# AhmedSalih3d/SPHExample

Hardware: AMD Instinct MI355X
Metric: particle-updates/sec (3D dam-break) (higher is better)
Workload: dtype f32

## Files before the change

sphexample_amd/csrc/sphmi_engine.hip:

```cpp
#include <hip/hip_runtime.h>

#include <algorithm>
#include <cmath>
#include <cstdio>
#include <cstring>
#include <limits>
#include <stdexcept>
#include <string>
#include <vector>

#include "../../include/sphmi.h"
#include "../../include/sphmi_internal.h"
#include "sphmi_kernels.h"
#include "sphmi_rebuild.h"

namespace sphmi {

struct EngineError : std::runtime_error {
    int status;
    EngineError(int s, const std::string& m) : std::runtime_error(m), status(s) {}
};

#define HC(expr)                                                                                   \
    do {                                                                                           \
// ... 220 lines not shown
        xcd_trace = getenv("SPHMI_XCD_TRACE") != nullptr;
        if (const char* w = getenv("SPHMI_TPB")) { const int v = atoi(w); if (v == 1 || v == 2 || v == 4) tpb = v; }
        if (const char* w = getenv("SPHMI_RESCHED")) resched = atoi(w);
        if (const char* w = getenv("SPHMI_TPB2")) tpb2 = atoi(w);
        if (const char* w = getenv("SPHMI_WPT2_BELOW")) kWptMedium = atoi(w);
        if (const char* w = getenv("SPHMI_CLASSES_FINE_BELOW")) classes_fine_below = atoi(w);
        HC(hipMalloc(&xcd_clock_d, 16 * 8)); HC(hipHostMalloc(&xcd_clock_h, 32 * 8));
        if (const char* w = getenv("SPHMI_XCD_SEGS")) { const int v = atoi(w); if (v >= 1 && v <= 4096) xcd_segs = v; }
        const size_t n = (size_t)N;
        for (int k = 0; k < 3; ++k) { HC(hipMalloc(&rec[k], 2 * n * sizeof(V4))); pk0[k] = Half<V4>(rec[k]); pk1[k] = Half<V4>(rec[k] + 1); }
        for (int k = 0; k < 2; ++k) {
            HC(hipMalloc(&acc[k], n * sizeof(V4)));
            HC(hipMalloc(&ghost[k], n * sizeof(V4))); HC(hipMemset(ghost[k], 0, n * sizeof(V4)));
            HC(hipMalloc(&type[k], n));
            HC(hipMalloc(&id[k], n * 8));
            HC(hipMalloc(&grp[k], n * 8));
            HC(hipMalloc(&key[k], n * 4));
            HC(hipMalloc(&prow[k], n * 4));
        }
        {
            const char* w = getenv("SPHMI_COMPENSATE");
            if (sizeof(T) == 4 && !(w && atoi(w) == 0))
                for (int k = 0; k < 2; ++k) { HC(hipMalloc(&comp[k], n * sizeof(V4))); HC(hipMemset(comp[k], 0, n * sizeof(V4))); }
        }
        HC(hipMalloc(&slot, n * 4)); HC(hipMalloc(&tmp_idx, n * 4)); HC(hipMalloc(&perm, n * 4));
        if (const char* w = getenv("SPHMI_POISON")) {
            const int b = atoi(w) & 255;
            for (int k = 0; k < 3; ++k) HC(hipMemset(rec[k], b, 2 * n * sizeof(V4)));
            for (int k = 0; k < 2; ++k) HC(hipMemset(acc[k], b, n * sizeof(V4)));
        }
        const size_t nt = n / kWave + 2;
        for (int k = 0; k < 2; ++k) { HC(hipMalloc(&tile_cost[k], nt * 4)); HC(hipMalloc(&tile_order[k], 8 * nt * 4)); }
        HC(hipMalloc(&tile_scan, nt * 4)); HC(hipMalloc(&tile_cls, nt)); HC(hipMalloc(&tile_work_d, nt * 4)); HC(hipMalloc(&tile_work1_d, nt * 4));
        if (cfg.kernel_output == SPHMI_KOUT_STORE) { HC(hipMalloc(&kout_d, n * sizeof(V4))); HC(hipMemset(kout_d, 0, n * sizeof(V4))); }
#if defined(SPHMI_STATS) || defined(SPHMI_TRACE)
        HC(hipMalloc(&trace_d, nt * 32 * 9)); HC(hipMemset(trace_d, 0, nt * 32 * 9));
#endif
        HC(hipMalloc(&tile_tsum, (nt / kScanTile + 2) * 4));
        static_assert(2 * sizeof(StepCtrl) <= kCtlRed, "control block layout");
        HC(hipMalloc(&ctl_d, kCtlBytes)); HC(hipMemset(ctl_d, 0, kCtlBytes)); HC(hipHostMalloc(&ctl_m, kCtlBytes)); memset(ctl_m, 0, kCtlBytes);
        ctrl_d = (StepCtrl*)ctl_d; red_d = (unsigned long long*)(ctl_d + kCtlRed); misc_d = (int*)(ctl_d + kCtlMisc); part_d = (int*)(ctl_d + kCtlPart);
        red_h = (unsigned long long*)(ctl_m + kCtlRed); misc_h = (int*)(ctl_m + kCtlMisc); part_h = (int*)(ctl_m + kCtlPart);
        HC(hipHostMalloc(&ctrl_h, sizeof(StepCtrl)));
        if (const char* w = getenv("SPHMI_FUSE_CTRL")) fuse_ctrl = atoi(w);
        if (const char* w = getenv("SPHMI_FUSE_MDBC")) fuse_mdbc = atoi(w);
        if (const char* w = getenv("SPHMI_SAME_CELLS")) same_cells = atoi(w);
        if (const char* w = getenv("SPHMI_DEVICE_REBUILD")) dev_rebuild = atoi(w);
        HC(hipMalloc(&bbox_d, 8 * 4));
        HC(hipHostMalloc(&bbox_h, 8 * 4));
    }
    ~Engine() override {
        (void)hipSetDevice(cfg.device);
        if (stream) (void)hipStreamSynchronize(stream);
        for (auto& e : ev_pool) { (void)hipEventDestroy(e.a); (void)hipEventDestroy(e.b); }
        for (auto& e : ev_pending) { (void)hipEventDestroy(e.a); (void)hipEventDestroy(e.b); }
        for (int k = 0; k < 3; ++k) (void)hipFree(rec[k]);
        for (int k = 0; k < 2; ++k) {
            (void)hipFree(acc[k]); (void)hipFree(ghost[k]); (void)hipFree(type[k]); (void)hipFree(id[k]); (void)hipFree(otag[k]);
            (void)hipFree(grp[k]); (void)hipFree(key[k]); (void)hipFree(prow[k]); (void)hipFree(comp[k]);
        }
        if (copy_stream) { (void)hipStreamSynchronize(copy_stream); (void)hipStreamDestroy(copy_stream); (void)hipEventDestroy(ev_packed); }
        for (auto& e : host_pinned) (void)hipHostUnregister(e.first);
        (void)hipFree(out_arena);
        (void)hipFree(slot); (void)hipFree(tmp_idx); (void)hipFree(perm);
        for (int k = 0; k < 2; ++k) { (void)hipFree(tile_cost[k]); (void)hipFree(tile_order[k]); }
        (void)hipFree(kout_d); (void)hipFree(tile_work_d); (void)hipFree(tile_work1_d); (void)hipFree(xcd_clock_d); (void)hipHostFree(xcd_clock_h);
        (void)hipFree(tile_scan); (void)hipFree(tile_cls); (void)hipFree(tile_tsum);
        (void)hipFree(count); (void)hipFree(cstart); (void)hipFree(tsum);
#if defined(SPHMI_STATS) || defined(SPHMI_TRACE)
        if (trace_d) {
            const char* fn = getenv("SPHMI_TRACE_FILE");
            std::vector<unsigned long long> tr((size_t)(cap / kWave + 2) * 4 * 9);
            if (fn && hipMemcpy(tr.data(), trace_d, tr.size() * 8, hipMemcpyDeviceToHost) == hipSuccess) {
                FILE* f = fopen(fn, "wb");
                if (f) { fwrite(tr.data(), 8, tr.size(), f); fclose(f); }
            }
            (void)hipFree(trace_d);
        }
#endif
#ifdef SPHMI_STATS
        {
            unsigned long long st[16];
            if (hipMemcpy(st, red_d, sizeof st, hipMemcpyDeviceToHost) == hipSuccess)
                fprintf(stderr, "[sphmi stats] wave-iterations %llu  lane-iterations %llu  refills %llu  empty refills %llu  chunks %llu  waves %llu\n",
                        st[8], st[9], st[10], st[11], st[12], st[13]);
        }
#endif
        (void)hipFree(ctl_d); (void)hipHostFree(ctl_m); (void)hipHostFree(ctrl_h); (void)hipFree(mdbc_list_d);
        (void)hipFree(bbox_d);
        (void)hipHostFree(bbox_h);
        (void)hipFree(cellx_d); (void)hipFree(uc_tsum);
        if (stream && own_stream) (void)hipStreamDestroy(stream);
    }

    static constexpr int kEvSample = 8;
    int ev_period = kEvSample;
    Ev begin_phase(int phase) {
        Ev e{};
        e.phase = phase; e.bstep = batch_step;
        e.weight = (phase == PH_REBUILD || phase == PH_REBUILD_DEVICE || iteration < ev_always_until) ? 1 : ((iteration % ev_period) == 0 ? ev_period : 0);
        if (e.weight == 0) return e;
        if (!ev_pool.empty()) { const int w = e.weight; e = ev_pool.back(); ev_pool.pop_back(); e.phase = phase; e.weight = w; e.bstep = batch_step; }
        else {
            HC(hipEventCreateWithFlags(&e.a, hipEventDisableSystemFence)); HC(hipEventCreateWithFlags(&e.b, hipEventDisableSystemFence));
        }
        HC(hipEventRecord(e.a, stream));
        return e;
    }
    void end_phase(Ev e) { if (e.weight == 0) return; HC(hipEventRecord(e.b, stream)); ev_pending.push_back(e); }
    void collect_events(int64_t executed = INT64_MAX) {
        for (auto& e : ev_pending) {
            float ms = 0;
            if (e.bstep >= 0 && e.bstep >= executed) { ev_pool.push_back(e); continue; }
            if (hipEventElapsedTime(&ms, e.a, e.b) == hipSuccess) {
                const bool edge = e.phase == PH_PASS1_EDGE || e.phase == PH_PASS2_EDGE;
                const int ph = e.phase == PH_PASS1_EDGE ? PH_PASS1 : (e.phase == PH_PASS2_EDGE ? PH_PASS2 : (e.phase == PH_REBUILD_DEVICE ? PH_REBUILD : e.phase));
                if (e.phase == PH_REBUILD_DEVICE) dev_rebuild_secs += ms * 1e-3;
                ph_secs[ph] += ms * 1e-3 * e.weight;
                ph_calls[ph] += edge ? 0 : e.weight;
                if (ph == PH_PASS1 || ph == PH_PASS2) { force_ms += ms * e.weight; force_launches += edge ? 0 : e.weight; }
            }
            ev_pool.push_back(e);
        }
        ev_pending.clear();
        if (force_launches > 0) {
            const double step_us = 2.0 * force_ms * 1e3 / (double)force_launches;
            ev_period = step_us >= 400.0 ? kEvSample : (step_us >= 100.0 ? 4 * kEvSample : 8 * kEvSample);
        }
    }

    static double decode(unsigned long long bits) {
        if constexpr (sizeof(T) == 4) { uint32_t u = (uint32_t)bits; float f; memcpy(&f, &u, 4); return (double)f; }
        else { double d; memcpy(&d, &bits, 8); return d; }
    }

    T kv2() const { return (T)(2.0 * cfg.m0 * cfg.alpha * cfg.c0 * cfg.h); }
    bool kv2_foldable() const { const T k = kv2(); return std::isnormal(k) && std::isfinite(T(1) / k) && std::isnormal(T(1) / k); }
    T cbe7() const { return (T)(((cfg.c0 * cfg.c0 * cfg.rho0) / 7.0) / std::pow(cfg.rho0, 7.0)); }
    bool eos_foldable() const { return sizeof(T) == 8 || (std::pow(4.0 * cfg.rho0, 7.0) < 1e37 && std::pow(0.25 * cfg.rho0, 7.0) > 1e-30 && std::isnormal(cbe7())); }
    bool compiled_in_model() const {
        return cfg.viscosity == SPHMI_VISC_ARTIFICIAL && cfg.density_diffusion == SPHMI_DDT_LINEAR && cfg.shifting == SPHMI_SHIFT_NONE &&
               cfg.kernel == SPHMI_KERNEL_WENDLAND_C2 && cfg.kernel_output == SPHMI_KOUT_NONE && kv2_foldable() && eos_foldable();
    }
    ForceParams<T> force_params(int src, int a, int out, double dt) const {
        ForceParams<T> P{};
        P.src0 = pk0[src]; P.src1 = pk1[src];
        P.a0 = pk0[a]; P.a1 = pk1[a];
        P.out0 = pk0[out]; P.out1 = pk1[out];
        P.accbuf = acc[cur]; P.comp = comp[cur];
        P.key = key[cur]; P.cstart = cstart; P.type = type[cur];
        P.red = red_cur(); P.stats = red_d + 8; P.ctrl = nullptr;
        P.N = N; P.nxp = grid.np[0]; P.nxyp = grid.np[0] * grid.np[1];
        P.dt = (T)dt; P.dt2 = (T)(dt * 0.5);
        P.H2 = (T)cfg.H2; P.h = (T)cfg.h; P.h_inv = (T)cfg.h_inv;
        P.Cgw = (T)(cfg.alphaD * 5.0 / (8.0 * cfg.h * cfg.h));
        P.Cfac = (T)(-8.0 * (cfg.alphaD * 5.0 / (8.0 * cfg.h * cfg.h))); P.nhinv_half = (T)(-0.5 * cfg.h_inv); P.big = (T)1099511627776.0;
        P.m0 = (T)cfg.m0;
        P.Kddt = (T)(cfg.delta_phi * cfg.h * cfg.c0 * cfg.m0);
        P.linfac = (T)(cfg.rho0 * cfg.g * ((1.0 / (cfg.Cb * cfg.gamma)) * cfg.rho0));
        P.eta2 = (T)std::max(cfg.eta2, 1e-24 * cfg.h * cfg.h);
        P.Kv2 = kv2();
        P.inv_Kv2 = kv2_foldable() ? T(1) / P.Kv2 : T(1);
        P.visc = cfg.viscosity; P.ddt = cfg.density_diffusion; P.shift = cfg.shifting == SPHMI_SHIFT_PLANAR;
        P.exact_cut = !(cfg.H >= 2.0 * cfg.h);
        P.kernel = cfg.kernel; P.kout = kout_d;
        P.alphaD = (T)cfg.alphaD; P.tens_eps = (T)cfg.cubic_eps;
        {
// ... 1347 lines not shown
```

sphexample_amd/csrc/sphmi_kernels.h:

```cpp
#pragma once
#include <hip/hip_runtime.h>
#include <stdint.h>
#include <type_traits>

namespace sphmi {

template <class T> struct Vec4;
template <> struct Vec4<float>  { using type = float4;  };
template <> struct Vec4<double> { using type = double4; };

template <class V> struct Half {
    V* p;
    __host__ __device__ Half() : p(nullptr) {}
    __host__ __device__ explicit Half(V* q) : p(q) {}
    template <class U> __host__ __device__ Half(const Half<U>& o) : p(o.p) {}
    __host__ __device__ V& operator[](long long i) const { return p[2 * i]; }
    __host__ __device__ explicit operator bool() const { return p != nullptr; }
};

constexpr int kWave = 64;
#ifndef SPHMI_LDS_STAGE
#define SPHMI_LDS_STAGE 0
#endif
#ifndef SPHMI_DIAG
// ... 212 lines not shown
}
__device__ __forceinline__ void atomic_max_bits(unsigned long long* p, float v, bool pretest = true) {
    unsigned int* q = reinterpret_cast<unsigned int*>(p);
    const unsigned int b = __float_as_uint(v);
    if (!pretest) { if (b != 0u) atomicMax(q, b); return; }
    if (b > __hip_atomic_load(q, __ATOMIC_RELAXED, __HIP_MEMORY_SCOPE_AGENT)) atomicMax(q, b);
}
__device__ __forceinline__ void atomic_max_bits(unsigned long long* p, double v, bool pretest = true) {
    const unsigned long long b = (unsigned long long)__double_as_longlong(v);
    if (!pretest) { if (b != 0ull) atomicMax(p, b); return; }
    if (b > __hip_atomic_load(p, __ATOMIC_RELAXED, __HIP_MEMORY_SCOPE_AGENT)) atomicMax(p, b);
}

typedef float f32x16 __attribute__((ext_vector_type(16)));
typedef unsigned u32x2 __attribute__((ext_vector_type(2)));
typedef _Float16 f16x8 __attribute__((ext_vector_type(8)));
typedef __fp16 h16x2 __attribute__((ext_vector_type(2)));
typedef unsigned u32x4s __attribute__((ext_vector_type(4)));
__device__ __forceinline__ unsigned pk_h2(float a, float b) { const h16x2 p = __builtin_amdgcn_cvt_pkrtz(a, b); return __builtin_bit_cast(unsigned, p); }
__device__ __forceinline__ float lo_half_as_float(unsigned p) { return (float)__builtin_bit_cast(h16x2, p)[0]; }
__device__ __forceinline__ unsigned split_hl(float v) { const unsigned h = pk_h2(v, 0.0f); return pk_h2(v, v - lo_half_as_float(h)); }
__device__ __forceinline__ void split_hh_ll(float v, unsigned& hh, unsigned& ll) { hh = pk_h2(v, v); const float r = v - lo_half_as_float(hh); ll = pk_h2(r, r); }

__device__ __forceinline__ void swap_halves(float& p, float& q) {
    const u32x2 r = __builtin_amdgcn_permlane32_swap(__float_as_uint(p), __float_as_uint(q), false, false);
    p = __uint_as_float(r[0]); q = __uint_as_float(r[1]);
}
__device__ __forceinline__ void swap_halves(unsigned& p, unsigned& q) {
    const u32x2 r = __builtin_amdgcn_permlane32_swap(p, q, false, false);
    p = r[0]; q = r[1];
}

__device__ __forceinline__ void wave_sync() {
    __builtin_amdgcn_fence(__ATOMIC_RELEASE, "wavefront");
    __builtin_amdgcn_wave_barrier();
    __builtin_amdgcn_fence(__ATOMIC_ACQUIRE, "wavefront");
}

template <class T, int D, int PASS, int MODEL, int WPT, int TPB = 1>
__global__ void __launch_bounds__(kWave * WPT * TPB)
__attribute__((amdgpu_waves_per_eu(1, 8)))
k_neighbor_force(const ForceParams<T> P) {
    static_assert(TPB == 1 || WPT <= 2, "several tiles per block: one or two waves per tile");
#if defined(SPHMI_STATS) || defined(SPHMI_TRACE)
    const unsigned long long st_entry = __builtin_amdgcn_s_memrealtime();
#endif
    T step_dt, step_dt2;
    if (PASS == PASS_PREDICTOR && P.ctl_in != nullptr) {
        StepCtrl c = *P.ctl_in;
        const unsigned long long r0 = P.red_in[0], r1 = P.red_in[1], r2 = P.red_in[2], r3 = P.red_in[3];
        const bool consumed = step_control_decide<T>(r0, r1, r2, r3, c, P.ctl_h, P.ctl_c0, P.ctl_CFL);
        if (blockIdx.x == 0 && threadIdx.x == 0) {
            *P.ctl_out = c;
            if (consumed) { P.red_zero[0] = 0; P.red_zero[1] = 0; P.red_zero[2] = 0; P.red_zero[3] = 0; }
        }
        if (!c.active) return;
        step_dt = (T)c.dt; step_dt2 = (T)c.dt2;
    } else {
        if (P.ctrl && !P.ctrl->active) return;
        if (PASS == PASS_PREDICTOR && P.mdbc_zero != nullptr && blockIdx.x == 0 && threadIdx.x == 0) {
            P.mdbc_zero[0] = 0; P.mdbc_zero[1] = 0; P.mdbc_zero[2] = 0; *P.mdbc_flag_zero = 0;
        }
        step_dt = P.ctrl ? (T)P.ctrl->dt : P.dt; step_dt2 = P.ctrl ? (T)P.ctrl->dt2 : P.dt2;
    }
    const int visc = MODEL >= 0 ? (MODEL & 15) : P.visc;
    const int ddt = MODEL >= 0 ? ((MODEL >> 4) & 15) : P.ddt;
    const bool shift = MODEL >= 0 ? false : (P.shift != 0 && PASS == PASS_CORRECTOR);
    using V4 = typename Vec4<T>::type;
    constexpr int NSEG = (D == 3) ? 9 : 3;
    constexpr int QCAP = queue_entries<T, WPT, MODEL>();
    constexpr int kQueueSlack = queue_slack<T, WPT, MODEL>();
    static_assert(QCAP >= 4 && kQueueSlack >= 1 && kQueueSlack <= QCAP - 1, "queue geometry");
    __shared__ uint2 s_q_all[SPHMI_LDS_STAGE ? 1 : WPT * TPB * QCAP * kWave];
    __shared__ V4 s_stage_all[SPHMI_LDS_STAGE ? WPT * TPB * 2 * kWave : 1];

    const int lane = threadIdx.x & (kWave - 1);
    const int wvb = threadIdx.x >> 6;
    const int tib = TPB == 1 ? 0 : wvb / WPT;
    const int wv = TPB == 1 ? wvb : (WPT == 1 ? 0 : ((wvb % WPT) ^ (int)((blockIdx.x >> 3) & 1)));
    uint2* const s_q = s_q_all + (SPHMI_LDS_STAGE ? 0 : wvb * QCAP * kWave + lane);
    [[maybe_unused]] V4* const s_stage = s_stage_all + (SPHMI_LDS_STAGE ? wvb * 2 * kWave : 0);
    constexpr bool kHalf = (WPT == 2 || WPT == 4 || WPT == 8) && SPHMI_LDS_STAGE == 0;
    constexpr int kPar = kHalf ? WPT / 2 : 1;
    constexpr bool kMixedExit = (kHalf && kPar > 1) || (!kHalf && WPT > 1 && TPB > 1);
    bool dead = false;
    int b;
    {
        const int x = blockIdx.x & 7, r = TPB == 1 ? (int)(blockIdx.x >> 3) : (int)(blockIdx.x >> 3) * TPB + tib;
        if (r >= P.part[8 + x]) {
            if constexpr (TPB == 1 || !kMixedExit) return;
            dead = true;
        }
        b = dead ? 0 : P.order[P.part[x] + r];
    }
    const int hl = kHalf ? (lane >> 5) : 0;
    const int half = kHalf ? (wv & 1) : 0;
    [[maybe_unused]] const int par = kHalf ? (wv >> 1) : 0;
    const int t0 = kHalf ? b * kWave + 32 * half : b * kWave;
    const int a = kHalf ? t0 + (lane & 31) : t0 + lane;
    const bool valid = a < P.N;
    const int ac = valid ? a : P.N - 1;
    const uint8_t ty_raw = P.type[ac];
    const bool owned = !dead && valid && !(ty_raw & 0xC0);
    unsigned long long owned_lanes = __builtin_amdgcn_ballot_w64(owned);
    if (owned_lanes == 0) {
        if constexpr (!kMixedExit) return;
        dead = true; owned_lanes = 1;
    }

    const V4 q0 = P.src0[ac];
    const V4 q1 = P.src1[ac];
    const T xa = q0.x, ya = q0.y, za = q0.z;
    T rho_a, rhon_a, P_a, s_a;
    if constexpr (PASS == PASS_CORRECTOR) {
        rho_a = q0.w;
        rhon_a = absT(q1.w);
        s_a = q1.w;
        P_a = eos7<T>(rho_a, P.rho0, P.inv_rho0, P.Cbe);
    } else {
        rho_a = absT(q0.w);
        rhon_a = rho_a;
        s_a = q0.w;
        P_a = q1.w;
    }
    constexpr bool kEarlyEpilogueLoads = PASS == PASS_CORRECTOR && WPT >= 4 && MODEL >= 0;
    [[maybe_unused]] V4 pre_s0, pre_s1, pre_lo;
    if constexpr (kEarlyEpilogueLoads) {
        pre_s0 = P.a0[ac]; pre_s1 = P.a1[ac];
        pre_lo.x = pre_lo.y = pre_lo.z = pre_lo.w = T(0);
        if (sizeof(T) == 4 && P.comp != nullptr) pre_lo = P.comp[ac];
    }
    const bool fluid_a = s_a > T(0);
    const T inv_rho_a = fast_rcp(rho_a);
    const T inv_rhon_a = (PASS == PASS_CORRECTOR) ? fast_rcp(rhon_a) : inv_rho_a;
    const T rm_a = rho_a * P.m0;
    constexpr bool kFoldKv2 = MODEL >= 0 && (MODEL & 15) == kViscArtificial && sizeof(T) == 4;
    const T c_a = kFoldKv2 ? -P.m0 * inv_rho_a * P.inv_Kv2 : -P.m0 * inv_rho_a;
    const T Kd_a = (ddt == kDdtZeroGravityLinear || fluid_a) ? T(-2) * P.Kddt : T(0);
    const T PaC = P_a - P.Cbe;

    const int key_a = P.key[ac];
    const int cs_a = P.cstart[key_a], ce_a = P.cstart[key_a + 1];
    const int last_lane = min(kHalf ? 31 : kWave - 1, P.N - 1 - t0);

    const int lane_o = __builtin_ctzll(owned_lanes);
    const T ox = rl(xa, lane_o), oy = rl(ya, lane_o), oz = rl(za, lane_o);
    const float txl = owned ? (float)(xa - ox) : 0.0f, tyl = owned ? (float)(ya - oy) : 0.0f, tzl = owned ? (float)(za - oz) : 0.0f;
    const float tt = txl * txl + tyl * tyl + tzl * tzl;
    float thr;
    {
        const float H2f = (float)P.H2;
        const float Rm = fast_sqrt(wave_max(owned ? tt : 0.0f)) + 6.0f * (float)P.h;
        const float eps = 1e-5f + 1e-6f * (Rm * Rm) / H2f;
        thr = owned ? H2f * (1.0f + eps) - tt : -1e30f;
    }
    [[maybe_unused]] const float m2x = -2.0f * txl, m2y = -2.0f * tyl, m2z = -2.0f * tzl;

    T drho = 0, ax = 0, ay = 0, az = 0;
    T gcx = 0, gcy = 0, gcz = 0, divr = 0;
    T kgx = 0, kgy = 0, kgz = 0, kw = 0;
    V4 vn_a = q1;
    if constexpr (PASS == PASS_CORRECTOR) { if (visc == kViscLaminarSPS) vn_a = P.a1[ac]; }

    const __amdgpu_buffer_rsrc_t rsA = __builtin_amdgcn_make_buffer_rsrc((void*)P.a0.p, 0, (int)((unsigned)P.N * 2u * (unsigned)sizeof(V4)), 0x00020000);
    T sum_c = 0, sum_d = 0;
    constexpr int kRecShift = sizeof(T) == 4 ? 5 : 6;
    auto rec_of = [](const unsigned m, const unsigned base) -> unsigned {
        const unsigned p = (unsigned)__builtin_ctz(m);
        if constexpr (kHalf) return ((p + (p & 0x1Cu)) << kRecShift) + base;
        else return (p << kRecShift) + base;
    };
    const unsigned cs_ar = (unsigned)cs_a << kRecShift, a_r1 = ((unsigned)a + 1u) << kRecShift, w_ai = ((unsigned)ce_a << kRecShift) - a_r1;
    auto pick_i = [&](const T if_i, const T if_j, const bool a_is_i) -> T { return a_is_i ? if_i : if_j; };
    auto pair_core = [&](const unsigned jr, const T dx, const T dy, const T dz, const T n0w, const V4& n1, const bool a_is_i) {
        const T r2 = (D == 3) ? dx * dx + dy * dy + dz * dz : dx * dx + dy * dy;
        T rho_b, rhon_b, s_b;
// ... 166 lines not shown
    const unsigned long long st_t0 = __builtin_amdgcn_s_memrealtime();
#endif
#ifdef SPHMI_STATS
    unsigned long long st_it = 0, st_lane = 0, st_ref = 0, st_emp = 0, st_chunks = 0;
#endif
    int work_it = 0, work_ch = 0;
    constexpr unsigned kEntryStride = kWave * 8, kQBytes = QCAP * kEntryStride;
    auto q_next = [](unsigned a) -> unsigned { a += kEntryStride; const unsigned b = a - kQBytes; return b < a ? b : a; };
    unsigned waddr = 0, raddr = 0;
    int qn = 0;
    unsigned cbase = 0;
    unsigned cm = 0;
    char* const s_qb = reinterpret_cast<char*>(s_q);
    constexpr bool kTwoPairs = WPT >= 8 || (WPT >= 4 && (MODEL >= 0 || D == 2));
    auto plays_i = [&](const unsigned jr) { return (bool)((jr < cs_ar) | ((jr - a_r1) < w_ai)); };
    auto run_pairs_plain = [&](const int keep, const bool drain, auto two_tag) __attribute__((always_inline)) {
        constexpr bool kTwo = decltype(two_tag)::value;
        unsigned qf = qn != 0 ? 1u : 0u;
        bool more = qn != 0, have = cm != 0;
        if (__builtin_amdgcn_ballot_w64(drain ? (more | have) : (qn > keep)) != 0) do {
            unsigned m = cm;
            if (cm < qf) {
                const uint2 ne = *reinterpret_cast<const uint2*>(s_qb + raddr);
                m = ne.x; raddr = q_next(raddr); qn -= 1;
                qf = min((unsigned)qn, 1u);
                cbase = ne.y;
            }
            work_it += 1;
#ifdef SPHMI_STATS
            st_it += 1; st_lane += __builtin_popcountll(__builtin_amdgcn_ballot_w64(m != 0));
#endif
            if constexpr (kTwo) {
                const unsigned m1 = m & (m - 1);
                cm = m1 & (m1 - 1);
                if (m != 0) {
                    const bool two = m1 != 0;
                    const unsigned jr0 = rec_of(m, cbase);
                    const unsigned jr1 = two ? rec_of(m1, cbase) : jr0;
                    const V4 n0a = gather_packet(rs0, jr0, 0, T());
                    const V4 n1a = gather_packet(rs0, jr0, 1, T());
                    const V4 n0b = gather_packet(rs0, jr1, 0, T());
                    const V4 n1b = gather_packet(rs0, jr1, 1, T());
                    pair(jr0, n0a, n1a, plays_i(jr0));
                    if (two) pair(jr1, n0b, n1b, plays_i(jr1));
                }
            } else {
                cm = m & (m - 1);
                if (m != 0) {
                    const unsigned jr = rec_of(m, cbase);
                    const V4 n0 = gather_packet(rs0, jr, 0, T());
                    const V4 n1 = gather_packet(rs0, jr, 1, T());
                    pair(jr, n0, n1, plays_i(jr));
                }
            }
            more = (qf | cm) != 0u; have = false;
        } while (__builtin_amdgcn_ballot_w64(drain ? (more | have) : (qn > keep)) != 0);
    };
    constexpr bool kPipe = (sizeof(T) == 4 || WPT == 2) && !kTwoPairs && SPHMI_LDS_STAGE == 0;
    [[maybe_unused]] bool pv = false;
    [[maybe_unused]] unsigned pjr = 0;
    constexpr bool kPairFetch64 = sizeof(T) == 8 && kHalf && MODEL >= 0 && SPHMI_DIAG == 0;
    [[maybe_unused]] const unsigned pf_c = (lane & 1) ? 16u : 0u, pf_self = a_r1 - (1u << kRecShift);
    auto run_pairs_piped = [&](const int keep, const bool drain) __attribute__((always_inline)) {
        unsigned qf = qn != 0 ? 1u : 0u;
        auto iteration = [&]() __attribute__((always_inline)) {
            work_it += 1;
#ifdef SPHMI_STATS
            st_it += 1; st_lane += __builtin_popcountll(__builtin_amdgcn_ballot_w64(pv));
#endif
            const unsigned jr = pjr;
            const bool v = pv;
            V4 n0, n1;
            [[maybe_unused]] u32x4_t A, B, Cq, Dq;
            if constexpr (kPairFetch64) {
                const unsigned js = v ? jr : pf_self;
                const unsigned jE = (unsigned)__builtin_amdgcn_mov_dpp((int)js, 0xA0, 0xF, 0xF, true) + pf_c;
                const unsigned jO = (unsigned)__builtin_amdgcn_mov_dpp((int)js, 0xF5, 0xF, 0xF, true) + pf_c;
                A = __builtin_amdgcn_raw_buffer_load_b128(rs0, (int)jE, 0, 0); B = __builtin_amdgcn_raw_buffer_load_b128(rs0, (int)(jE + 32u), 0, 0);
                Cq = __builtin_amdgcn_raw_buffer_load_b128(rs0, (int)jO, 0, 0); Dq = __builtin_amdgcn_raw_buffer_load_b128(rs0, (int)(jO + 32u), 0, 0);
            } else
#if SPHMI_DIAG == 2 || SPHMI_DIAG == 4
            if (v) { n0 = q0; n1 = q1; n0.x += __uint_as_float(jr) * T(1e-30); n0.y += T(0.003); n0.w = q0.w + T(1); }
#else
            { if (v) { n0 = gather_packet(rs0, jr, 0, T()); n1 = gather_packet(rs0, jr, 1, T()); } }
#endif
            unsigned m = cm;
            if (cm < qf) {
                const uint2 ne = *reinterpret_cast<const uint2*>(s_qb + raddr);
                m = ne.x; raddr = q_next(raddr); qn -= 1;
                if constexpr (sizeof(T) == 4) asm("v_min_u32 %0, %1, 1" : "=v"(qf) : "v"(qn));
                else qf = min((unsigned)qn, 1u);
                cbase = ne.y;
            }
            cm = m & (m - 1);
            pv = m != 0;
            pjr = rec_of(m, cbase);
            if constexpr (kPairFetch64) {
                unsigned w[16];
#define SPHMI_PF(d, x, y) "v_cndmask_b32_dpp %" #d ", %" #x ", %" #y ", vcc quad_perm:[1,0,3,2] row_mask:0xf bank_mask:0xf bound_ctrl:1\n\t"
                asm volatile("s_mov_b32 vcc_lo, 0x55555555\n\ts_mov_b32 vcc_hi, 0x55555555\n\ts_nop 1\n\t"
                             SPHMI_PF(0, 16, 8) SPHMI_PF(1, 17, 9) SPHMI_PF(2, 18, 10) SPHMI_PF(3, 19, 11)
                             SPHMI_PF(4, 20, 12) SPHMI_PF(5, 21, 13) SPHMI_PF(6, 22, 14) SPHMI_PF(7, 23, 15)
                             : "=&v"(w[0]), "=&v"(w[1]), "=&v"(w[2]), "=&v"(w[3]), "=&v"(w[8]), "=&v"(w[9]), "=&v"(w[10]), "=&v"(w[11])
                             : "v"(A.x), "v"(A.y), "v"(A.z), "v"(A.w), "v"(B.x), "v"(B.y), "v"(B.z), "v"(B.w),
                               "v"(Cq.x), "v"(Cq.y), "v"(Cq.z), "v"(Cq.w), "v"(Dq.x), "v"(Dq.y), "v"(Dq.z), "v"(Dq.w) : "vcc");
                asm volatile("s_mov_b32 vcc_lo, 0xaaaaaaaa\n\ts_mov_b32 vcc_hi, 0xaaaaaaaa\n\ts_nop 1\n\t"
                             SPHMI_PF(0, 8, 16) SPHMI_PF(1, 9, 17) SPHMI_PF(2, 10, 18) SPHMI_PF(3, 11, 19)
                             SPHMI_PF(4, 12, 20) SPHMI_PF(5, 13, 21) SPHMI_PF(6, 14, 22) SPHMI_PF(7, 15, 23)
                             : "=&v"(w[4]), "=&v"(w[5]), "=&v"(w[6]), "=&v"(w[7]), "=&v"(w[12]), "=&v"(w[13]), "=&v"(w[14]), "=&v"(w[15])
                             : "v"(A.x), "v"(A.y), "v"(A.z), "v"(A.w), "v"(B.x), "v"(B.y), "v"(B.z), "v"(B.w),
                               "v"(Cq.x), "v"(Cq.y), "v"(Cq.z), "v"(Cq.w), "v"(Dq.x), "v"(Dq.y), "v"(Dq.z), "v"(Dq.w) : "vcc");
#undef SPHMI_PF
                auto dbl = [](unsigned lo, unsigned hi) { return __longlong_as_double((long long)(((unsigned long long)hi << 32) | lo)); };
                n0.x = dbl(w[0], w[1]); n0.y = dbl(w[2], w[3]); n0.z = dbl(w[4], w[5]); n0.w = dbl(w[6], w[7]);
                n1.x = dbl(w[8], w[9]); n1.y = dbl(w[10], w[11]); n1.z = dbl(w[12], w[13]); n1.w = dbl(w[14], w[15]);
            }
            if (v) pair(jr, n0, n1, plays_i(jr));
        };
        if (__builtin_amdgcn_ballot_w64(drain ? (pv | ((qf | cm) != 0u)) : (qn > keep)) != 0) do {
            iteration();
            if constexpr (sizeof(T) == 4) iteration();
        } while (__builtin_amdgcn_ballot_w64(drain ? (pv | ((qf | cm) != 0u)) : (qn > keep)) != 0);
    };
    constexpr bool kPipe2 = kTwoPairs && SPHMI_LDS_STAGE == 0 && MODEL >= 0;
    [[maybe_unused]] bool pv2 = false;
    [[maybe_unused]] unsigned pjr2 = 0;
    auto run_pairs_piped2 = [&](const int keep, const bool drain) __attribute__((always_inline)) {
        unsigned qf = qn != 0 ? 1u : 0u;
        if (__builtin_amdgcn_ballot_w64(drain ? (pv | ((qf | cm) != 0u)) : (qn > keep)) != 0) do {
            work_it += 1;
#ifdef SPHMI_STATS
            st_it += 1; st_lane += __builtin_popcountll(__builtin_amdgcn_ballot_w64(pv)) + __builtin_popcountll(__builtin_amdgcn_ballot_w64(pv2));
#endif
            const unsigned jr0 = pjr, jr1 = pjr2;
            const bool v0 = pv, v1 = pv2;
            V4 n0a, n1a, n0b, n1b;
            if (v0) {
                n0a = gather_packet(rs0, jr0, 0, T()); n1a = gather_packet(rs0, jr0, 1, T());
                n0b = gather_packet(rs0, jr1, 0, T()); n1b = gather_packet(rs0, jr1, 1, T());
            }
            unsigned m = cm;
            if (cm < qf) {
                const uint2 ne = *reinterpret_cast<const uint2*>(s_qb + raddr);
                m = ne.x; raddr = q_next(raddr); qn -= 1;
                qf = min((unsigned)qn, 1u);
                cbase = ne.y;
            }
            const unsigned m1 = m & (m - 1);
            cm = m1 & (m1 - 1);
            pv = m != 0; pv2 = m1 != 0;
            pjr = rec_of(m, cbase);
            pjr2 = pv2 ? rec_of(m1, cbase) : pjr;
            if (v0) {
                pair(jr0, n0a, n1a, plays_i(jr0));
                if (v1) pair(jr1, n0b, n1b, plays_i(jr1));
            }
        } while (__builtin_amdgcn_ballot_w64(drain ? (pv | ((qf | cm) != 0u)) : (qn > keep)) != 0);
    };
    auto run_pairs = [&](const int keep, const bool drain) __attribute__((always_inline)) {
        if constexpr (kPipe2) run_pairs_piped2(keep, drain);
        else if constexpr (kPipe) run_pairs_piped(keep, drain);
        else run_pairs_plain(keep, drain, std::bool_constant<kTwoPairs>());
    };

    const int bperm = kHalf ? lane : (((lane >> 2) & 1) << 5) | ((lane >> 5) << 4) | (((lane >> 3) & 3) << 2) | (lane & 3);
    float B0[2], B1[2], B2[2], A2;
    if constexpr (kHalf) {
// ... 34 lines not shown
        for (int C = 1; C >= 0; --C) {
            if (C == 1 && HI - cb <= 32) continue;
            u32x4s aw; aw[0] = C ? Z[0] : X[0]; aw[1] = C ? Z[1] : X[1]; aw[2] = C ? Z[2] : X[2]; aw[3] = C ? Z[3] : X[3];
            f32x16 d = {0};
            d = __builtin_amdgcn_mfma_f32_32x32x16_f16(__builtin_bit_cast(f16x8, aw), __builtin_bit_cast(f16x8, Bh), d, 0, 0, 0);
#pragma unroll
            for (int r = 15; r >= 0; --r)
                W = __builtin_amdgcn_alignbit(W, __float_as_uint(d[r]), 31);
            __builtin_amdgcn_sched_barrier(0);
        }
        return (unsigned long long)W;
    };
    auto chunk_packet = [&](const int cb, const int HI) -> V4 {
        const int c = cb + bperm;
        if constexpr (kHalf) return gather_packet(rs0, (unsigned)c << kRecShift, 0, T());
        else return P.src0[c < HI ? c : cb];
    };
    auto scan_chunk = [&](const int cb, const int HI, const V4& cpk) -> unsigned long long {
        const int c = cb + bperm;
        const bool cv = c < HI;
        float A0[2], A1[2];
        A0[0] = (float)(cpk.x - ox); A0[1] = (float)(cpk.y - oy); A1[0] = (float)(cpk.z - oz);
        A1[1] = cv ? A0[0] * A0[0] + A0[1] * A0[1] + A1[0] * A1[0] : 1e30f;
        swap_halves(A0[0], A0[1]);
        swap_halves(A1[0], A1[1]);
        unsigned W[2] = {0u, 0u};
#pragma unroll
        for (int C = 1; C >= 0; --C) {
            if (kHalf && C == 1 && HI - cb <= 32) continue;
#pragma unroll
            for (int Tb = 0; Tb < (kHalf ? 1 : 2); ++Tb) {
                f32x16 d = {0};
                d = __builtin_amdgcn_mfma_f32_32x32x2f32(A0[C], B0[Tb], d, 0, 0, 0);
                d = __builtin_amdgcn_mfma_f32_32x32x2f32(A1[C], B1[Tb], d, 0, 0, 0);
                d = __builtin_amdgcn_mfma_f32_32x32x2f32(A2, B2[Tb], d, 0, 0, 0);
#pragma unroll
                for (int r = 15; r >= 0; --r)
                    W[Tb] = __builtin_amdgcn_alignbit(W[Tb], __float_as_uint(d[r]), 31);
                __builtin_amdgcn_sched_barrier(0);
            }
        }
        if constexpr (kHalf) return (unsigned long long)W[0];
        swap_halves(W[0], W[1]);
        return ((unsigned long long)W[1] << 32) | W[0];
    };

    int g0 = 0;
    auto row_offset = [&](const int seg) { return (D == 3) ? ((seg % 3) - 1) * P.nxp + ((seg / 3) - 1) * P.nxyp : (seg - 1) * P.nxp; };
    constexpr bool kShareRanges = WPT >= 4 && !kHalf;
    __shared__ int2 s_rng[kShareRanges ? NSEG * kWave : 1];
    constexpr bool kPrefetchRanges = WPT >= 4 && kHalf && MODEL >= 0;
    __shared__ int2 s_rng_own[kPrefetchRanges ? WPT * TPB * NSEG * kWave : 1];
    [[maybe_unused]] int2* const s_rng_w = s_rng_own + (kPrefetchRanges ? wvb * NSEG * kWave + lane : 0);
    if constexpr (kShareRanges) {
#pragma unroll
        for (int k = 0; k < (NSEG + WPT - 1) / WPT; ++k) {
            const int seg = wv + k * WPT;
            if (seg < NSEG) {
                const int off = row_offset(seg);
                s_rng[seg * kWave + lane] = make_int2(valid ? P.cstart[key_a + off - 1] : 0, valid ? P.cstart[key_a + off + 2] : 0);
            }
        }
        __syncthreads();
    }
    [[maybe_unused]] int bal = 0;
    auto push_entry = [&](const unsigned bits, const int c0) {
        if (bits != 0) {
            *reinterpret_cast<uint2*>(s_qb + waddr) = make_uint2(bits, (unsigned)c0 << kRecShift); waddr = q_next(waddr); qn += 1;
        }
    };
    const int nseg = dead ? 0 : NSEG;
    if constexpr (kPrefetchRanges) {
        if (!dead) {
            int2 rg[NSEG];
#pragma unroll
            for (int seg = 0; seg < NSEG; ++seg) {
                const int off = row_offset(seg);
                rg[seg] = make_int2(valid ? P.cstart[key_a + off - 1] : 0, valid ? P.cstart[key_a + off + 2] : 0);
            }
#pragma unroll
            for (int seg = 0; seg < NSEG; ++seg) s_rng_w[seg * kWave] = rg[seg];
        }
    }
#pragma unroll 1
    for (int seg = 0; seg < nseg; ++seg) {
        int lo_l, hi_l;
        if constexpr (kShareRanges) { const int2 rg = s_rng[seg * kWave + lane]; lo_l = rg.x; hi_l = rg.y; }
        else if constexpr (kPrefetchRanges) { const int2 rg = s_rng_w[seg * kWave]; lo_l = rg.x; hi_l = rg.y; }
        else {
            const int off = row_offset(seg);
            lo_l = valid ? P.cstart[key_a + off - 1] : 0;
            hi_l = valid ? P.cstart[key_a + off + 2] : 0;
        }
        const int LO = rl_i(lo_l, 0);
        const int HI = rl_i(hi_l, last_lane);
        [[maybe_unused]] int row_b0 = 0, row_b1 = 0;
        if constexpr (kHalf) {
            auto below = [](const int X) -> int { return 4 * (X >> 3) + min(X & 7, 4); };
            row_b0 = below(lo_l - LO - 4 * hl); row_b1 = below(hi_l - LO - 4 * hl);
        }
        int first = 0;
        if constexpr (WPT > 1 && !kHalf) {
            if constexpr (WPT >= 4) first = (wv - g0) & (WPT - 1);
            else first = (wv + WPT - seg % WPT) % WPT;
            g0 = (g0 + (HI > LO ? (HI - LO + kWave - 1) / kWave : 0)) & (WPT - 1);
        }
        if constexpr (kHalf && kPar > 1) first = (par + seg) & (kPar - 1);
#pragma unroll 1
        for (int cb = LO + first * kWave; cb < HI; cb += kHalf ? kWave * kPar : kWave * WPT) {
            if (__builtin_amdgcn_ballot_w64((lo_l < cb + kWave) & (hi_l > cb)) == 0) continue;
            if (__builtin_amdgcn_ballot_w64(qn > QCAP - 2) != 0) run_pairs(QCAP - 1 - kQueueSlack, false);
            unsigned long long m;
            {
                const V4 cpk = chunk_packet(cb, HI);
                if constexpr (kHalf) m = scan_chunk16(cb, HI, cpk);
                else m = scan_chunk(cb, HI, cpk);
                if constexpr (kHalf) {
                    const int t = (cb - LO) >> 1;
                    const int b0 = min(max(row_b0 - t, 0), 32), b1 = min(max(row_b1 - t, 0), 32);
                    const int w = b1 - b0;
                    const unsigned rm = ((~0u) >> ((32 - w) & 31)) << (b0 & 31);
                    m = (w > 0) ? (unsigned long long)((unsigned)m & rm) : 0ull;
                } else {
                const int b0 = max(lo_l - cb, 0), b1 = min(hi_l - cb, 64);
                const int w = b1 - b0;
                const unsigned long long rm = ((~0ull) >> ((64 - w) & 63)) << (b0 & 63);
                m = (w > 0) ? (m & rm) : 0ull;
                }
            }
            work_ch += 1;
#ifdef SPHMI_STATS
            st_chunks += 1;
#endif
#if SPHMI_LDS_STAGE
            {
                const int c = cb + lane;
                const bool cvs = c < HI;
                const V4 s0 = P.src0[cvs ? c : cb], s1 = P.src1[cvs ? c : cb];
                wave_sync();
                s_stage[2 * lane] = s0; s_stage[2 * lane + 1] = s1;
                wave_sync();
                unsigned long long mm = m;
                while (__builtin_amdgcn_ballot_w64(mm != 0ull) != 0) {
                    work_it += 1;
#ifdef SPHMI_STATS
                    st_it += 1; st_lane += __builtin_popcountll(__builtin_amdgcn_ballot_w64(mm != 0ull));
#endif
                    if (mm != 0ull) {
                        const int b = __builtin_ctzll(mm);
                        mm &= mm - 1ull;
                        const V4 n0 = s_stage[2 * b], n1 = s_stage[2 * b + 1];
                        const unsigned jr = (unsigned)(cb + b) << kRecShift;
                        pair(jr, n0, n1, plays_i(jr));
                    }
                }
                continue;
            }
#endif
            if constexpr (kHalf) {
                unsigned wl = (unsigned)m, wu = (unsigned)m;
                swap_halves(wl, wu);
                const int cl = __builtin_popcount(wl), cu = __builtin_popcount(wu);
                const bool lower_takes_upper = (bal <= 0) != (cl >= cu);
                const int d = lower_takes_upper ? cu - cl : cl - cu;
                bal += d;
                const bool take_upper = lower_takes_upper != (hl != 0);
                push_entry(take_upper ? wu : wl, cb + (take_upper ? 4 : 0));
            } else { push_entry((unsigned)m, cb); push_entry((unsigned)(m >> 32), cb + 32); }
// ... 188 lines not shown
```

Before: 1.294 billion.

## Stage a 256-record neighbour window in LDS and serve in-window gathers from it

For the default f32 3D predictor/corrector model with WPT=2, TPB=2, each block cooperatively loads a 256-particle window of packed source records around its (possibly adjacent) tiles into shared memory. Neighbour gathers that fall inside the window read from LDS instead of issuing global buffer loads. The segment loop is rotated to start at the centre row so window hits come first. This adds 8 KB of LDS per block, a __syncthreads, and a per-lane branch, which may reduce occupancy and add divergence between LDS and global fetch paths.

New measurement: 1.371 billion (median of 6 runs). 1.06x the previous value.

```diff
diff --git a/sphexample_amd/csrc/sphmi_engine.hip b/sphexample_amd/csrc/sphmi_engine.hip
--- a/sphexample_amd/csrc/sphmi_engine.hip
+++ b/sphexample_amd/csrc/sphmi_engine.hip
@@ -326,7 +326,7 @@
         {
             unsigned long long st[16];
             if (hipMemcpy(st, red_d, sizeof st, hipMemcpyDeviceToHost) == hipSuccess)
-                fprintf(stderr, "[sphmi stats] wave-iterations %llu  lane-iterations %llu  refills %llu  empty refills %llu  chunks %llu  waves %llu\n",
+                fprintf(stderr, "[sphmi stats] wave-iterations %llu  lane-iterations %llu  window pairs %llu  gather-free iterations %llu  chunks %llu  waves %llu\n",
                         st[8], st[9], st[10], st[11], st[12], st[13]);
         }
 #endif
diff --git a/sphexample_amd/csrc/sphmi_kernels.h b/sphexample_amd/csrc/sphmi_kernels.h
--- a/sphexample_amd/csrc/sphmi_kernels.h
+++ b/sphexample_amd/csrc/sphmi_kernels.h
@@ -318,7 +318,10 @@
     [[maybe_unused]] V4* const s_stage = s_stage_all + (SPHMI_LDS_STAGE ? wvb * 2 * kWave : 0);
     constexpr bool kHalf = (WPT == 2 || WPT == 4 || WPT == 8) && SPHMI_LDS_STAGE == 0;
     constexpr int kPar = kHalf ? WPT / 2 : 1;
-    constexpr bool kMixedExit = (kHalf && kPar > 1) || (!kHalf && WPT > 1 && TPB > 1);
+    constexpr bool kWindow = sizeof(T) == 4 && D == 3 && PASS != PASS_FORCES_ONLY && MODEL == kModelDefault && WPT == 2 && TPB == 2 &&
+                             SPHMI_LDS_STAGE == 0;
+    constexpr int kWinRecords = 256;
+    constexpr bool kMixedExit = (kHalf && kPar > 1) || (!kHalf && WPT > 1 && TPB > 1) || kWindow;
     bool dead = false;
     int b;
     {
@@ -328,6 +331,21 @@
             dead = true;
         }
         b = dead ? 0 : P.order[P.part[x] + r];
+    }
+    __shared__ V4 s_win[kWindow ? 2 * kWinRecords : 1];
+    [[maybe_unused]] unsigned win_r = 0u, win_len = 0u;
+    [[maybe_unused]] V4 win0, win1;
+    if constexpr (kWindow) {
+        const int x = blockIdx.x & 7, r0 = (int)(blockIdx.x >> 3) * TPB, n = P.part[8 + x];
+        if (r0 >= n) return;
+        const int b0 = P.order[P.part[x] + r0], b1 = r0 + 1 < n ? P.order[P.part[x] + r0 + 1] : -2;
+        const bool adjacent = b1 == b0 + 1 || b1 == b0 - 1;
+        const int w0 = max(0, min(adjacent ? kWave * min(b0, b1) - kWave : kWave * b0 - 96, P.N - kWinRecords));
+        win_r = (unsigned)w0 << 5;
+        win_len = (adjacent || tib == 0) ? (unsigned)(kWinRecords * 32) : 0u;
+        const unsigned g = (unsigned)(w0 + kWave * wvb + lane) << 5;
+        const __amdgpu_buffer_rsrc_t rsw = __builtin_amdgcn_make_buffer_rsrc((void*)P.src0.p, 0, (int)((unsigned)P.N * 2u * (unsigned)sizeof(V4)), 0x00020000);
+        win0 = gather_packet(rsw, g, 0, T()); win1 = gather_packet(rsw, g, 1, T());
     }
     const int hl = kHalf ? (lane >> 5) : 0;
     const int half = kHalf ? (wv & 1) : 0;
@@ -660,7 +678,20 @@
 #if SPHMI_DIAG == 2 || SPHMI_DIAG == 4
             if (v) { n0 = q0; n1 = q1; n0.x += __uint_as_float(jr) * T(1e-30); n0.y += T(0.003); n0.w = q0.w + T(1); }
 #else
-            { if (v) { n0 = gather_packet(rs0, jr, 0, T()); n1 = gather_packet(rs0, jr, 1, T()); } }
+            if constexpr (kWindow) {
+                const unsigned wo = jr - win_r;
+                const bool in_win = wo < win_len;
+#ifdef SPHMI_STATS
+                st_ref += __builtin_popcountll(__builtin_amdgcn_ballot_w64(v && in_win));
+                st_emp += (__builtin_amdgcn_ballot_w64(v && !in_win) == 0 && __builtin_amdgcn_ballot_w64(v) != 0) ? 1 : 0;
+#endif
+                if (v) {
+                    if (in_win) {
+                        const char* const w = reinterpret_cast<const char*>(s_win) + wo;
+                        n0 = *reinterpret_cast<const V4*>(w); n1 = *reinterpret_cast<const V4*>(w + 16);
+                    } else { n0 = gather_packet(rs0, jr, 0, T()); n1 = gather_packet(rs0, jr, 1, T()); }
+                }
+            } else { if (v) { n0 = gather_packet(rs0, jr, 0, T()); n1 = gather_packet(rs0, jr, 1, T()); } }
 #endif
             unsigned m = cm;
             if (cm < qf) {
@@ -861,8 +892,14 @@
             for (int seg = 0; seg < NSEG; ++seg) s_rng_w[seg * kWave] = rg[seg];
         }
     }
+    if constexpr (kWindow) {
+        V4* const w = s_win + 2 * (kWave * wvb + lane);
+        w[0] = win0; w[1] = win1;
+        __syncthreads();
+    }
 #pragma unroll 1
-    for (int seg = 0; seg < nseg; ++seg) {
+    for (int s = 0; s < nseg; ++s) {
+        const int seg = kWindow ? (s + NSEG / 2) % NSEG : s;
         int lo_l, hi_l;
         if constexpr (kShareRanges) { const int2 rg = s_rng[seg * kWave + lane]; lo_l = rg.x; hi_l = rg.y; }
         else if constexpr (kPrefetchRanges) { const int2 rg = s_rng_w[seg * kWave]; lo_l = rg.x; hi_l = rg.y; }
```
